# Roywangj/AdaptPoint

Hardware: AMD Instinct MI355X
Metric: set-abstraction fwd+bwd point-clouds/sec (B=32,N=1024) (higher is better)
Workload: dtype bf16

## Files before the change

### adaptpoint_amd/csrc/ball_query_body.h

```cpp
#pragma once
#include "apn_common.h"

namespace apn {

constexpr int BQ_CHUNK = 4096;
constexpr int BQ_QPW = 4;

template <int WAVES, int QPW = BQ_QPW>
__device__ __forceinline__ void ball_query_body(
    int n, int m, float radius2, int nsample, int q_per_block, int zero_empty,
    const float *__restrict__ new_xyz, const float *__restrict__ xyz, int *__restrict__ idx,
    int cloud, int bx, float *s_dyn) {
    const int chunk = min(n, BQ_CHUNK);
    float *sx = s_dyn, *sy = s_dyn + chunk, *sz = s_dyn + 2 * chunk;
    int *s_cnt = reinterpret_cast<int *>(s_dyn + 3 * chunk);

    const int tid = threadIdx.x;
    const int lane = tid & 63;
    const int wave = __builtin_amdgcn_readfirstlane(tid >> 6);
    const int q_begin = bx * q_per_block;
    const int q_end = min(q_begin + q_per_block, m);

    xyz += (size_t)cloud * n * 3;
    new_xyz += (size_t)cloud * m * 3;
    idx += (size_t)cloud * m * nsample;

    int *cnt_of = s_cnt;
    int *first_of = s_cnt + q_per_block;
    for (int i = tid; i < q_per_block; i += WAVES * 64) { cnt_of[i] = 0; first_of[i] = 0; }

    for (int base = 0; base < n; base += BQ_CHUNK) {
        const int len = min(BQ_CHUNK, n - base);
        __syncthreads();
        for (int i = tid; i < 3 * len; i += WAVES * 64) {
            const float v = xyz[(size_t)base * 3 + i];
            const int p = i / 3, c = i - p * 3;
            (c == 0 ? sx : c == 1 ? sy : sz)[p] = v;
        }
        __syncthreads();

        for (int qb = q_begin + wave * QPW; qb < q_end; qb += WAVES * QPW) {
            int cnt[QPW], first[QPW];
            float qx[QPW], qy[QPW], qz[QPW];
            bool open = false;
#pragma unroll
            for (int j = 0; j < QPW; ++j) {
                const int q = qb + j;
                const bool in = q < q_end;
                cnt[j] = in ? __builtin_amdgcn_readfirstlane(cnt_of[q - q_begin]) : nsample;
                first[j] = in ? __builtin_amdgcn_readfirstlane(first_of[q - q_begin]) : 0;
                const int qc = in ? q : q_begin;
                qx[j] = new_xyz[qc * 3 + 0];
                qy[j] = new_xyz[qc * 3 + 1];
                qz[j] = new_xyz[qc * 3 + 2];
                open = open || cnt[j] < nsample;
            }
            if (!open) continue;
            for (int k0 = 0; k0 < len; k0 += 64) {
                const int k = k0 + lane;
                const bool inside = k < len;
                const float px = inside ? sx[k] : 0.0f, py = inside ? sy[k] : 0.0f, pz = inside ? sz[k] : 0.0f;
                bool any_open = false;
#pragma unroll
                for (int j = 0; j < QPW; ++j) {
                    if (cnt[j] >= nsample) continue;
                    const bool hit = inside && dist2(qx[j] - px, qy[j] - py, qz[j] - pz) < radius2;
                    const unsigned long long mask = __ballot(hit);
                    if (mask != 0ull) {
                        if (cnt[j] == 0) first[j] = base + k0 + (int)__builtin_ctzll(mask);
                        const int slot = cnt[j] + (int)__builtin_amdgcn_mbcnt_hi(
                                                      (unsigned)(mask >> 32),
                                                      __builtin_amdgcn_mbcnt_lo((unsigned)mask, 0u));
                        if (hit && slot < nsample) idx[(size_t)(qb + j) * nsample + slot] = base + k;
                        cnt[j] += (int)__builtin_popcountll(mask);
                    }
                    any_open = any_open || cnt[j] < nsample;
                }
                if (!any_open) break;
            }
            if (lane == 0) {
#pragma unroll
                for (int j = 0; j < QPW; ++j)
                    if (qb + j < q_end) { cnt_of[qb + j - q_begin] = cnt[j]; first_of[qb + j - q_begin] = first[j]; }
            }
        }
    }

    __syncthreads();
    for (int q = q_begin + wave; q < q_end; q += WAVES) {
        const int ql = q - q_begin;
        const int cnt = __builtin_amdgcn_readfirstlane(cnt_of[ql]);
        if ((cnt == 0 && !zero_empty) || cnt >= nsample) continue;
        const int first = __builtin_amdgcn_readfirstlane(first_of[ql]);
        int *row = idx + (size_t)q * nsample;
        for (int l = cnt + lane; l < nsample; l += 64) row[l] = first;
    }
}


}
```

Before: 121,000.

## Cache ball-query candidate points in registers and process queries one at a time

Restructures ball query so each wave keeps up to 1024 candidate points in per-lane registers (16 slots), loaded lazily in groups of 4, and reuses them across all queries it handles. This avoids re-reading LDS for every query. Queries are now processed one at a time with the next query's coordinates prefetched. The padding fill is done inline when the last chunk finishes, which removes the final barrier and the shared-memory count/first bookkeeping when n fits in registers. The cost is higher VGPR pressure, which can lower occupancy, and more complex control flow.

```diff
diff --git a/adaptpoint_amd/csrc/ball_query_body.h b/adaptpoint_amd/csrc/ball_query_body.h
--- a/adaptpoint_amd/csrc/ball_query_body.h
+++ b/adaptpoint_amd/csrc/ball_query_body.h
@@ -5,6 +5,11 @@
 
 constexpr int BQ_CHUNK = 4096;
 constexpr int BQ_QPW = 4;
+constexpr int BQ_SLOTS = 16;
+constexpr int BQ_REG = 64 * BQ_SLOTS;
+constexpr int BQ_GROUP = 4;
+
+__device__ __forceinline__ int opaque_v(int v) { asm volatile("" : "+v"(v)); return v; }
 
 template <int WAVES, int QPW = BQ_QPW>
 __device__ __forceinline__ void ball_query_body(
@@ -25,9 +30,18 @@
     new_xyz += (size_t)cloud * m * 3;
     idx += (size_t)cloud * m * nsample;
 
+    const bool carried = n > BQ_REG;
     int *cnt_of = s_cnt;
     int *first_of = s_cnt + q_per_block;
-    for (int i = tid; i < q_per_block; i += WAVES * 64) { cnt_of[i] = 0; first_of[i] = 0; }
+    if (carried)
+        for (int i = tid; i < q_per_block; i += WAVES * 64) { cnt_of[i] = 0; first_of[i] = 0; }
+
+    auto finish = [&](int q, int cnt, int first) {
+        if ((cnt == 0 && !zero_empty) || cnt >= nsample) return;
+        int *row = idx + (size_t)q * nsample;
+#pragma nounroll
+        for (int l = cnt + lane; l < nsample; l += 64) row[l] = first;
+    };
 
     for (int base = 0; base < n; base += BQ_CHUNK) {
         const int len = min(BQ_CHUNK, n - base);
@@ -39,62 +53,84 @@
         }
         __syncthreads();
 
-        for (int qb = q_begin + wave * QPW; qb < q_end; qb += WAVES * QPW) {
-            int cnt[QPW], first[QPW];
-            float qx[QPW], qy[QPW], qz[QPW];
-            bool open = false;
+        for (int rc = 0; rc < len; rc += BQ_REG) {
+            const int rlen = min(BQ_REG, len - rc);
+            const bool last = base + rc + BQ_REG >= n;
+            const int point0 = base + rc + lane;
+            float px[BQ_SLOTS], py[BQ_SLOTS], pz[BQ_SLOTS];
 #pragma unroll
-            for (int j = 0; j < QPW; ++j) {
-                const int q = qb + j;
-                const bool in = q < q_end;
-                cnt[j] = in ? __builtin_amdgcn_readfirstlane(cnt_of[q - q_begin]) : nsample;
-                first[j] = in ? __builtin_amdgcn_readfirstlane(first_of[q - q_begin]) : 0;
-                const int qc = in ? q : q_begin;
-                qx[j] = new_xyz[qc * 3 + 0];
-                qy[j] = new_xyz[qc * 3 + 1];
-                qz[j] = new_xyz[qc * 3 + 2];
-                open = open || cnt[j] < nsample;
-            }
-            if (!open) continue;
-            for (int k0 = 0; k0 < len; k0 += 64) {
-                const int k = k0 + lane;
-                const bool inside = k < len;
-                const float px = inside ? sx[k] : 0.0f, py = inside ? sy[k] : 0.0f, pz = inside ? sz[k] : 0.0f;
-                bool any_open = false;
+            for (int s = 0; s < BQ_SLOTS; ++s) px[s] = py[s] = pz[s] = __builtin_nanf("");
+            int loaded = 0;
+
+#pragma nounroll
+            for (int qb = q_begin + wave * QPW; qb < q_end; qb += WAVES * QPW) {
+                const int qe = min(qb + QPW, q_end);
+                float nx = new_xyz[qb * 3 + 0], ny = new_xyz[qb * 3 + 1], nz = new_xyz[qb * 3 + 2];
+#pragma nounroll
+                for (int q = qb; q < qe; ++q) {
+                    const float qx = nx, qy = ny, qz = nz;
+                    const int qn = min(q + 1, qe - 1);
+                    nx = new_xyz[qn * 3 + 0]; ny = new_xyz[qn * 3 + 1]; nz = new_xyz[qn * 3 + 2];
+                    int cnt = 0, first = 0;
+                    if (carried) {
+                        cnt = __builtin_amdgcn_readfirstlane(cnt_of[q - q_begin]);
+                        first = __builtin_amdgcn_readfirstlane(first_of[q - q_begin]);
+                    }
+                    if (cnt < nsample) {
+                        int *row = idx + (size_t)q * nsample;
+                        const bool empty = cnt == 0;
+                        int rel = 0;
 #pragma unroll
-                for (int j = 0; j < QPW; ++j) {
-                    if (cnt[j] >= nsample) continue;
-                    const bool hit = inside && dist2(qx[j] - px, qy[j] - py, qz[j] - pz) < radius2;
-                    const unsigned long long mask = __ballot(hit);
-                    if (mask != 0ull) {
-                        if (cnt[j] == 0) first[j] = base + k0 + (int)__builtin_ctzll(mask);
-                        const int slot = cnt[j] + (int)__builtin_amdgcn_mbcnt_hi(
-                                                      (unsigned)(mask >> 32),
-                                                      __builtin_amdgcn_mbcnt_lo((unsigned)mask, 0u));
-                        if (hit && slot < nsample) idx[(size_t)(qb + j) * nsample + slot] = base + k;
-                        cnt[j] += (int)__builtin_popcountll(mask);
+                        for (int g = 0; g < BQ_SLOTS / BQ_GROUP; ++g) {
+                            if (g * BQ_GROUP * 64 >= rlen) break;
+                            if (loaded == g) {
+#pragma unroll
+                                for (int t = 0; t < BQ_GROUP; ++t) {
+                                    const int s = g * BQ_GROUP + t;
+                                    const int k = 64 * s + opaque_v(lane);
+                                    const int kc = rc + min(k, rlen - 1);
+                                    const float vx = sx[kc], vy = sy[kc], vz = sz[kc];
+                                    if (k < rlen) { px[s] = vx; py[s] = vy; pz[s] = vz; }
+                                }
+                                loaded = g + 1;
+                            }
+                            bool hit[BQ_GROUP];
+                            unsigned long long mask[BQ_GROUP];
+#pragma unroll
+                            for (int t = 0; t < BQ_GROUP; ++t) {
+                                const int s = g * BQ_GROUP + t;
+                                hit[t] = dist2(qx - px[s], qy - py[s], qz - pz[s]) < radius2;
+                                mask[t] = __ballot(hit[t]);
+                            }
+#pragma unroll
+                            for (int t = 0; t < BQ_GROUP; ++t) {
+                                if (mask[t] == 0ull) continue;
+                                const int s = g * BQ_GROUP + t;
+                                if (cnt == 0) rel = 64 * s + (int)__builtin_ctzll(mask[t]);
+                                const int slot = cnt + (int)__builtin_amdgcn_mbcnt_hi(
+                                                           (unsigned)(mask[t] >> 32),
+                                                           __builtin_amdgcn_mbcnt_lo((unsigned)mask[t], 0u));
+                                if (hit[t] && slot < nsample)
+                                    *reinterpret_cast<int *>(reinterpret_cast<char *>(row) + (unsigned)slot * 4u) = opaque_v(point0) + 64 * s;
+                                cnt += (int)__builtin_popcountll(mask[t]);
+                            }
+                            if (cnt >= nsample) break;
+                        }
+                        if (empty && cnt > 0) first = base + rc + rel;
                     }
-                    any_open = any_open || cnt[j] < nsample;
+                    if (last) {
+                        finish(q, cnt, first);
+                    } else if (lane == 0) {
+                        cnt_of[q - q_begin] = cnt;
+                        first_of[q - q_begin] = first;
+                    }
                 }
-                if (!any_open) break;
-            }
-            if (lane == 0) {
-#pragma unroll
-                for (int j = 0; j < QPW; ++j)
-                    if (qb + j < q_end) { cnt_of[qb + j - q_begin] = cnt[j]; first_of[qb + j - q_begin] = first[j]; }
             }
         }
     }
 
-    __syncthreads();
-    for (int q = q_begin + wave; q < q_end; q += WAVES) {
-        const int ql = q - q_begin;
-        const int cnt = __builtin_amdgcn_readfirstlane(cnt_of[ql]);
-        if ((cnt == 0 && !zero_empty) || cnt >= nsample) continue;
-        const int first = __builtin_amdgcn_readfirstlane(first_of[ql]);
-        int *row = idx + (size_t)q * nsample;
-        for (int l = cnt + lane; l < nsample; l += 64) row[l] = first;
-    }
+    if (n == 0)
+        for (int q = q_begin + wave; q < q_end; q += WAVES) finish(q, 0, 0);
 }
 
 
```

Result: faster. 123,000 (median of 6 runs) (+1.6%).
